# phuang1024/Starst3r

Hardware: AMD Instinct MI355X
Metric: 3DGS train iters/sec @ 1M Gaussians, 8x1080p views (higher is better)
Workload: dtype f32

## Files before the change

### starst3r_amd/csrc/adam.hip

```cpp
#include "per_view.h"

struct AdamK {
    float step_size, bc2_sqrt, w1, w2, b2, eps;
};

#define ADAM_SKIP(count_dev, count_cap, status_dev) \
    (((count_dev) && (uint32_t)(count_dev)[0] > (count_cap)) || ((status_dev) && (status_dev)[0] != 0))

__device__ __forceinline__ float* adam_param(int64_t i, int64_t N, float* means, float* quats, float* scales,
                                             float* opacities, float* sh, int sh_stride) {
    if (i < 3 * N) return means + i;
    if (i < 7 * N) return quats + (i - 3 * N);
    if (i < 10 * N) return scales + (i - 7 * N);
    if (i < 11 * N) return opacities + (i - 10 * N);
    const int64_t j = i - 11 * N;
    const int64_t g = j / 12;
    return sh + g * sh_stride + (j - g * 12);
}

__global__ __launch_bounds__(256) void k_adam(int64_t N, float* __restrict__ means, float* __restrict__ quats,
                                              float* __restrict__ scales, float* __restrict__ opacities,
                                              float* __restrict__ sh, int sh_stride,
                                              const float* __restrict__ grads, float* __restrict__ m,
                                              float* __restrict__ v, AdamK k, const int32_t* __restrict__ count_dev,
                                              uint32_t count_cap, const int32_t* __restrict__ status_dev, int64_t i0,
                                              int64_t i1, int64_t g0, int64_t g1,
                                              float* __restrict__ pstage, const float* __restrict__ gstage,
                                              float* __restrict__ grads_out) {
    if (ADAM_SKIP(count_dev, count_cap, status_dev)) return;
    const bool by_gaussian = g1 - g0 < N || gstage;
    const int64_t n = g1 - g0;
    const int64_t total = by_gaussian ? 23 * n : i1 - i0;
    const int64_t stride = (int64_t)gridDim.x * blockDim.x;
    for (int64_t j = (int64_t)blockIdx.x * blockDim.x + threadIdx.x; j < total; j += stride) {
        int64_t i;
        if (by_gaussian) {
            if (j < 3 * n) i = 3 * g0 + j;
            else if (j < 7 * n) i = 3 * N + 4 * g0 + (j - 3 * n);
            else if (j < 10 * n) i = 7 * N + 3 * g0 + (j - 7 * n);
            else if (j < 11 * n) i = 10 * N + g0 + (j - 10 * n);
            else i = 11 * N + 12 * g0 + (j - 11 * n);
        } else {
            i = i0 + j;
        }
        float* p = adam_param(i, N, means, quats, scales, opacities, sh, sh_stride);
        float gi;
        if (gstage) { gi = gstage[23 * g0 + j]; grads_out[i] = gi; }
        else gi = grads[i];
        const float mi = fmaf(k.w1, gi - m[i], m[i]);
        const float vi = v[i] * k.b2 + (k.w2 * gi) * gi;
        m[i] = mi; v[i] = vi;
        const float denom = sqrtf(vi) / k.bc2_sqrt + k.eps;
        const float pn = *p - k.step_size * (mi / denom);
        *p = pn;
        if (pstage) pstage[i] = pn;
    }
}

__global__ __launch_bounds__(256) void k_adam4(int64_t N, float* __restrict__ means, float* __restrict__ quats,
                                               float* __restrict__ scales, float* __restrict__ opacities,
                                               float* __restrict__ sh, int sh_stride,
                                               const float* __restrict__ grads, float* __restrict__ m,
                                               float* __restrict__ v, AdamK k, const int32_t* __restrict__ count_dev,
                                               uint32_t count_cap, const int32_t* __restrict__ status_dev, int64_t i0,
                                               int64_t i1, float* __restrict__ pstage) {
    if (ADAM_SKIP(count_dev, count_cap, status_dev)) return;
    const int64_t total4 = (i1 - i0) >> 2;
    const int64_t stride = (int64_t)gridDim.x * blockDim.x;
    for (int64_t j = (int64_t)blockIdx.x * blockDim.x + threadIdx.x; j < total4; j += stride) {
        const int64_t i = i0 + 4 * j;
        float4* p = reinterpret_cast<float4*>(adam_param(i, N, means, quats, scales, opacities, sh, sh_stride));
        const float4 g4 = *reinterpret_cast<const float4*>(grads + i);
        float4 m4 = *reinterpret_cast<float4*>(m + i), v4 = *reinterpret_cast<float4*>(v + i), p4 = *p;
        const float gi[4] = {g4.x, g4.y, g4.z, g4.w};
        float mi[4] = {m4.x, m4.y, m4.z, m4.w}, vi[4] = {v4.x, v4.y, v4.z, v4.w}, pi[4] = {p4.x, p4.y, p4.z, p4.w};
#pragma unroll
        for (int q = 0; q < 4; ++q) {
            mi[q] = fmaf(k.w1, gi[q] - mi[q], mi[q]);
            vi[q] = vi[q] * k.b2 + (k.w2 * gi[q]) * gi[q];
            const float denom = sqrtf(vi[q]) / k.bc2_sqrt + k.eps;
            pi[q] = pi[q] - k.step_size * (mi[q] / denom);
        }
        *reinterpret_cast<float4*>(m + i) = make_float4(mi[0], mi[1], mi[2], mi[3]);
        *reinterpret_cast<float4*>(v + i) = make_float4(vi[0], vi[1], vi[2], vi[3]);
        const float4 pn = make_float4(pi[0], pi[1], pi[2], pi[3]);
        *p = pn;
        if (pstage) *reinterpret_cast<float4*>(pstage + i) = pn;
    }
}

__global__ __launch_bounds__(256) void k_params_from_stage(int64_t N, float* __restrict__ means, float* __restrict__ quats,
                                                           float* __restrict__ scales, float* __restrict__ opacities,
                                                           float* __restrict__ sh, int sh_stride,
                                                           const float* __restrict__ pstage, int64_t i0, int64_t i1,
                                                           int64_t lim, const int32_t* __restrict__ count_dev,
                                                           uint32_t count_cap, const int32_t* __restrict__ status_dev) {
    if (ADAM_SKIP(count_dev, count_cap, status_dev)) return;
    const int64_t stride = (int64_t)gridDim.x * blockDim.x;
    for (int64_t i = (int64_t)blockIdx.x * blockDim.x + threadIdx.x; i < lim; i += stride) {
        if (i >= i0 && i < i1) continue;
        *adam_param(i, N, means, quats, scales, opacities, sh, sh_stride) = pstage[i];
    }
}

__global__ __launch_bounds__(256) void k_params_from_peers(int64_t N, float* __restrict__ means, float* __restrict__ quats,
                                                           float* __restrict__ scales, float* __restrict__ opacities,
                                                           float* __restrict__ sh, int sh_stride,
                                                           const float* const* __restrict__ tab, int r, int64_t q,
                                                           int64_t lim, const int32_t* __restrict__ status_dev) {
    if (status_dev && status_dev[0] != 0) return;
    const int64_t stride = (int64_t)gridDim.x * blockDim.x;
    for (int64_t i = (int64_t)blockIdx.x * blockDim.x + threadIdx.x; i < lim; i += stride) {
        const int p = (int)(i / q);
        if (p == r) continue;
        *adam_param(i, N, means, quats, scales, opacities, sh, sh_stride) =
            __uint_as_float(__hip_atomic_load(reinterpret_cast<const unsigned*>(tab[p] + i), __ATOMIC_RELAXED, __HIP_MEMORY_SCOPE_SYSTEM));
    }
}

int st3r_params_from_peers_impl(hipStream_t s, int N, float* means, float* quats, float* scales, float* opacities,
                                float* sh, int sh_stride, const float* const* tab, int r, int64_t q, int64_t lim,
                                const int32_t* status_dev) {
    if (lim <= 0 || q <= 0) return ST3R_OK;
    int blocks = ceil_div(lim, 256);
    if (blocks > 256 * 16) blocks = 256 * 16;
    hipLaunchKernelGGL(k_params_from_peers, dim3(blocks), dim3(256), 0, s, (int64_t)N, means, quats, scales, opacities, sh,
                       sh_stride, tab, r, q, lim, status_dev);
    LAUNCH_CHECK();
    return ST3R_OK;
}

static AdamK adam_constants(double lr, double b1, double b2, double eps, int step) {
    AdamK k;
    const double bc1 = 1.0 - pow(b1, (double)step), bc2 = 1.0 - pow(b2, (double)step);
    k.step_size = (float)(lr / bc1);
    k.bc2_sqrt = (float)sqrt(bc2);
    k.w1 = (float)(1.0 - b1); k.w2 = (float)(1.0 - b2); k.b2 = (float)b2; k.eps = (float)eps;
    return k;
}

int st3r_adam_impl(hipStream_t s, int N, float* means, float* quats, float* scales, float* opacities, float* sh,
                   int sh_stride, const float* grads, float* m, float* v, double lr, double b1, double b2,
                   double eps, int step, const int32_t* count_dev, uint32_t count_cap, const int32_t* status_dev, int64_t i0,
                   int64_t i1, int64_t g0, int64_t g1, float* pstage, const float* gstage, float* grads_out) {
    if (N == 0) return ST3R_OK;
    if (i0 < 0) { i0 = 0; i1 = 23 * (int64_t)N; }
    if (g1 < 0) { g0 = 0; g1 = N; }
    const AdamK k = adam_constants(lr, b1, b2, eps, step);
    const int64_t total = (g1 - g0 < N) ? 23 * (g1 - g0) : i1 - i0;
    if (total <= 0) return ST3R_OK;
    const bool contiguous = !(g1 - g0 < N) && !gstage;
#ifndef ADAM_NO_VEC
    if (contiguous && N % 4 == 0 && i0 % 4 == 0 && (i1 - i0) % 4 == 0 && sh_stride % 4 == 0 &&
        aligned16(means, quats, scales, opacities, sh, grads, m, v, pstage)) {
        int blocks4 = ceil_div(total / 4, 256);
        if (blocks4 > 256 * 16) blocks4 = 256 * 16;
        hipLaunchKernelGGL(k_adam4, dim3(blocks4), dim3(256), 0, s, (int64_t)N, means, quats, scales, opacities, sh,
                           sh_stride, grads, m, v, k, count_dev, count_cap, status_dev, i0, i1, pstage);
        LAUNCH_CHECK();
        return ST3R_OK;
    }
#endif
    int blocks = ceil_div(total, 256);
    if (blocks > 256 * 16) blocks = 256 * 16;
    hipLaunchKernelGGL(k_adam, dim3(blocks), dim3(256), 0, s, (int64_t)N, means, quats, scales, opacities, sh,
                       sh_stride, grads, m, v, k, count_dev, count_cap, status_dev, i0, i1, g0, g1, pstage, gstage, grads_out);
    LAUNCH_CHECK();
    return ST3R_OK;
}

int st3r_params_from_stage_impl(hipStream_t s, int N, float* means, float* quats, float* scales, float* opacities,
// ... 54 lines not shown
```

### starst3r_amd/csrc/comm.hip

```cpp
#include <dlfcn.h>

#include <vector>

#include <rccl/rccl.h>

#include <chrono>
#include <thread>

#include "stages.h"

namespace {
struct RcclApi {
    void* handle;
    ncclResult_t (*get_unique_id)(ncclUniqueId*);
    ncclResult_t (*comm_init_rank)(ncclComm_t*, int, ncclUniqueId, int);
    ncclResult_t (*comm_destroy)(ncclComm_t);
    ncclResult_t (*all_reduce)(const void*, void*, size_t, ncclDataType_t, ncclRedOp_t, ncclComm_t, hipStream_t);
    ncclResult_t (*reduce_scatter)(const void*, void*, size_t, ncclDataType_t, ncclRedOp_t, ncclComm_t, hipStream_t);
    ncclResult_t (*all_gather)(const void*, void*, size_t, ncclDataType_t, ncclComm_t, hipStream_t);
    ncclResult_t (*group_start)();
    ncclResult_t (*group_end)();
    const char* (*get_error_string)(ncclResult_t);
};

// ... 319 lines not shown
    }
    __syncthreads();
    if (p == 0 && status_out) *status_out = accumulate ? (*status_out | s_any) : s_any;
    __threadfence_system();
}

__device__ __forceinline__ float peer_load(const float* p) {
    return __uint_as_float(__hip_atomic_load(reinterpret_cast<const unsigned*>(p), __ATOMIC_RELAXED, __HIP_MEMORY_SCOPE_SYSTEM));
}
__global__ __launch_bounds__(256) void k_xreduce(const float* const* __restrict__ grad_tab, int w, int r, int64_t i0,
                                                 int64_t i1, int64_t t0, int64_t t1, float* __restrict__ out) {
    const int64_t n = (i1 - i0) + (t1 - t0);
    const int64_t stride = (int64_t)gridDim.x * blockDim.x;
    for (int64_t j = (int64_t)blockIdx.x * blockDim.x + threadIdx.x; j < n; j += stride) {
        const int64_t i = j < i1 - i0 ? i0 + j : t0 + (j - (i1 - i0));
        float acc = 0.f;
        for (int p = 0; p < w; ++p) {
            const float v = p == r ? grad_tab[p][i] : peer_load(grad_tab[p] + i);
            acc = p == 0 ? v : acc + v;
        }
        out[i] = acc;
    }
}

ST3R_EXPORT int st3r_gs_train_step(st3r_ctx* ctx, void* stream, int N, int C, float* means, float* quats, float* scales,
                                   float* opacities, float* sh, int sh_stride, const float* viewmats, const float* Ks,
                                   const float* campos, const float* gt_images, int width, int height, float ssim_fac,
                                   float opac_fac, float scale_fac, float* grads, float* m, float* v, double lr,
                                   double beta1, double beta2, double eps, int step, float* loss_out,
                                   int64_t* stats_host) {
    ARG_CHECK(ctx && grads && m && v && step >= 1 && N > 0);
    hipStream_t s = (hipStream_t)stream;
    if (!ctx->comm) {
        int rc = st3r_gs_train_fwd_bwd(ctx, stream, N, C, means, quats, scales, opacities, sh, sh_stride, viewmats, Ks,
                                       campos, gt_images, width, height, ssim_fac, opac_fac, scale_fac, grads, loss_out,
                                       stats_host);
        if (rc) return rc;
        return st3r_adam_step(ctx, stream, N, means, quats, scales, opacities, sh, sh_stride, grads, m, v, lr, beta1, beta2,
                              eps, step);
    }
    RcclApi* api = rccl_api();
    if (!api) return ST3R_ERR_HIP;
    ncclComm_t comm = (ncclComm_t)ctx->comm;
    int rc = st3r_peer_status_settle(ctx);
    if (rc) return rc;
    if (ctx->comm_broken) {
        st3r_set_error("this communicator lost lockstep in an earlier step (a device-side barrier timed out): no further "
                       "step is exchanged over it");
        return ST3R_ERR_PEER;
    }
    const int mode = ctx->exchange;
    int32_t* counts = nullptr;
    rc = st3r_counts_buffer(ctx, s, &counts);
    if (rc) return rc;
    if (!ctx->peer_event) HIP_TRY(hipEventCreateWithFlags(&ctx->peer_event, hipEventDisableTiming));
    const int K = (mode == ST3R_EXCHANGE_RANGES && N >= 4096) ? EXCH_RANGES_K : 1;
    if (mode == ST3R_EXCHANGE_RANGES) {
        rc = ensure_comm_stream(ctx);
        if (rc) return rc;
        ctx->n_ranges = K;
    }
    XWindow* xw = nullptr;
    if (mode == ST3R_EXCHANGE_DIRECT) {
        rc = xwin_ensure(ctx, api, s, (int64_t)23 * N);
        if (rc) return rc;
        xw = (XWindow*)ctx->xwin;
    }
    float* const grads_local = xw ? xw->grad : grads;
    int rc_local = (ctx->debug_flags & 2048)
                       ? (st3r_set_error("debug flag 2048: simulated failure of this rank's step"), ST3R_ERR_NOMEM)
// ... 129 lines not shown
```

### starst3r_amd/csrc/fused_step.hip

```cpp
#include "radix_sort.h"
#include "stages.h"

int st3r_count_settle(st3r_ctx* ctx) {
    if (!ctx->count_pending) return ST3R_OK;
    HIP_TRY(hipEventSynchronize(ctx->count_event));
    ctx->count_pending = 0;
    const int64_t n = (int64_t)((int32_t*)(ctx->pinned + 8))[0];
    if (n < 0) {
        ctx->isect_hint = 0;
        ctx->view_chunks = (ctx->view_chunks > 0 ? ctx->view_chunks : 1) * 2;
        st3r_set_error("the previous step produced more than 2^31 tile intersections: its gradients were incomplete -- "
                       "repeat it (st3r_gs_train_fwd_bwd / st3r_gs_train_step now walk the views in %d chunks)",
                       ctx->view_chunks);
        return ST3R_ERR_CAPACITY;
    }
    if (n > ctx->count_cap) {
        ctx->isect_hint = 0;
        st3r_set_error("the previous step produced %lld tile intersections, more than the %lld its buffers were sized "
                       "for from the step before (+25 %%): its gradients were incomplete and st3r_adam_step / "
                       "st3r_gs_train_step did NOT apply them (the update is guarded on the device) -- repeat that step",
                       (long long)n, (long long)ctx->count_cap);
        return ST3R_ERR_CAPACITY;
    }
    ctx->isect_hint = n;
// ... 228 lines not shown
        rc = st3r_loss_impl(ctx, s, ro.C, ro.H, ro.W, ex.exposure ? im.exposed : im.rgb, b.gt, 1.0f - ssim_fac, ssim_fac,
                            b.sums, im.v_rgb, sums_cleared, lw);
    if (!rc && ex.exposure)
        rc = st3r_exposure_bwd_impl(ctx, s, ro.C, ro.H, ro.W, im.rgb, ex.exposure, im.v_rgb, im.v_rgb, ex.v_exposure);
    if (!rc && dp.prior)
        rc = st3r_depth_prior_loss_impl(ctx, s, ro.C, ro.H, ro.W, im.depth, im.alpha, dp.prior, dp.weight, dp.norm, 1, dp.fac,
                                        b.dp_sums, 1, im.v_depth, im.v_alpha);
    st3r_prof_end(ctx, s, STG_LOSS);
    return rc;
}

static int blend_backward(st3r_ctx* ctx, hipStream_t s, const RasterOut& ro, const StepImages& im, bool need_pairs,
                          st3r_vtile_ref* slots, float* v_pairs) {
    RasterOut rb = ro;
    if (ctx->debug_flags & 2) { rb.rects = nullptr; rb.rectbase = nullptr; }
    const bool eio = true;
    st3r_prof_begin(ctx, s, STG_BLEND_BWD);
    int rc = st3r_blend_bwd_impl(ctx, s, rb, im.alpha, im.last, im.v_rgb, im.v_alpha, nullptr, eio, slots);
    if (!rc && need_pairs) {
        ARENA_GET(SLOT_VSPLATS_D, float, ro.n_pairs * ST3R_SPLAT_STRIDE, v_pairs_d);
        rc = st3r_blend_depth_bwd_impl(ctx, s, rb, im.alpha, im.last, im.v_depth, v_pairs_d, eio);
        if (!rc) {
            if (slots->vtile) rc = st3r_gather_vtile_impl(s, ro.n_pairs, slots, v_pairs);
            else HIP_TRY(hipMemsetAsync(v_pairs, 0, sizeof(float) * ST3R_SPLAT_STRIDE * (size_t)ro.n_pairs, s));
        }
        if (!rc) rc = st3r_add_pairs_impl(s, ro.n_pairs, v_pairs, v_pairs_d);
    }
    st3r_prof_end(ctx, s, STG_BLEND_BWD);
    return rc;
}

static int project_backward(st3r_ctx* ctx, hipStream_t s, const GsParams& g, const GsViews& v, const RasterOut& ro,
                            const LossFacs& f, const float* v_pairs, const st3r_vtile_ref* slots, bool accumulate,
                            float* grads) {
    ctx->ranges_recorded = 0;
    if (!(ctx->n_ranges > 1 && ctx->comm_stream))
        return st3r_project_sh_bwd_impl(s, g, v, 0.3f, ro.splats, v_pairs, (float)v.C, f.opac, f.scale, grads, accumulate, 0,
                                        -1, false, slots);
    ARENA_GET(SLOT_GSTAGE, float, (int64_t)23 * g.N, gstage);
    const int K = ctx->n_ranges;
    for (int j = 0; j < K; ++j) {
        const int g0 = (int)((int64_t)g.N * j / K), g1 = (int)((int64_t)g.N * (j + 1) / K);
        int rc = st3r_project_sh_bwd_impl(s, g, v, 0.3f, ro.splats, v_pairs, (float)v.C, f.opac, f.scale, gstage, accumulate,
                                          g0, g1, true, slots);
        if (rc) return rc;
        HIP_TRY(hipEventRecord(ctx->ev_range_bwd[j], s));
    }
    ctx->ranges_recorded = K;
    return ST3R_OK;
}

static int pose_backward(st3r_ctx* ctx, hipStream_t s, const GsParams& g, const GsViews& v, const RasterOut& ro,
                         const float* v_pairs, float* v_viewmats) {
    return st3r_gs_viewmat_bwd(ctx, s, g.N, v.C, g.means, g.quats, g.scales, g.sh, g.sh_stride, v.viewmats, v.Ks, v.campos,
                               v.W, v.H, 0.3f, ro.splats, v_pairs, v_viewmats);
}

static int train_views(st3r_ctx* ctx, hipStream_t s, const GsParams& g, const ViewBatch& b, const LossFacs& f,
                       double* reg_sums, bool allow_async, bool accumulate, float* grads, RasterOut* ro_out) {
    const GsViews& v = b.v;
    DepthPrior dp{};
    int rc = b.dp_sums ? st3r_depth_prior_for(ctx, s, b.gt, v.C, v.H, v.W, &dp) : ST3R_OK;
    if (rc) return rc;
    ExposureReg ex{};
    if (b.exposure) st3r_exposure_for(ctx, b.gt, v.C, v.H, v.W, &ex);
    LossWeight lw{};
    if (b.weighted) rc = st3r_loss_weight_for(ctx, s, b.gt, v.C, v.H, v.W, &lw);
    if (rc) return rc;
    const bool need_pairs = dp.prior != nullptr;
    RasterOut& ro = *ro_out;
    rc = rasterize_front(ctx, s, g, v, reg_sums, 1, nullptr, allow_async, &ro, b.sums);
    if (rc) return rc;
    StepImages im;
    rc = step_images(ctx, ro, need_pairs, ex.exposure != nullptr, &im);
    if (rc) return rc;
    float* const v_Ks = st3r_intrinsics_grad_for(ctx, b.gt, v.C, v.H, v.W);
    float* v_pairs = nullptr;
    if (need_pairs || b.v_viewmats || v_Ks) {
        ARENA_GET(SLOT_VSPLATS, float, ro.n_pairs * ST3R_SPLAT_STRIDE, vp);
        v_pairs = vp;
    }
    rc = forward_and_losses(ctx, s, ro, b, f.ssim, true, dp, ex, lw, im);
    if (rc) return rc;
    st3r_vtile_ref slots{};
    rc = blend_backward(ctx, s, ro, im, need_pairs, &slots, v_pairs);
    if (rc) return rc;
    st3r_prof_begin(ctx, s, STG_PROJECT_BWD);
    rc = project_backward(ctx, s, g, v, ro, f, need_pairs ? v_pairs : nullptr, need_pairs ? nullptr : &slots, accumulate,
                          grads);
    if (!rc && need_pairs && b.v_viewmats) rc = pose_backward(ctx, s, g, v, ro, v_pairs, b.v_viewmats);
    if (!rc && need_pairs) rc = st3r_gs_depth_bwd(ctx, s, g.N, v.C, g.means, v.viewmats, ro.splats, v_pairs, grads, b.v_viewmats);
    st3r_prof_end(ctx, s, STG_PROJECT_BWD);
    if (!rc && !need_pairs && (b.v_viewmats || v_Ks)) {
        rc = st3r_gather_vtile_impl(s, ro.n_pairs, &slots, v_pairs);
        if (!rc && b.v_viewmats) rc = pose_backward(ctx, s, g, v, ro, v_pairs, b.v_viewmats);
    }
    if (!rc && v_Ks)
        rc = st3r_gs_intrinsics_bwd(ctx, s, g.N, v.C, g.means, g.quats, g.scales, v.viewmats, v.Ks, v.W, v.H, 0.3f,
                                    ro.splats, v_pairs, v_Ks);
    return rc;
}

static int train_chunks(st3r_ctx* ctx, hipStream_t s, const GsParams& g, const ViewBatch& all, const LossFacs& f,
                        double* reg_sums, double* reg_scratch, bool want_stats, float* grads, int* chunks, int64_t stats[3]) {
    const int C = all.v.C;
    for (;;) {
        int rc = ST3R_OK;
        stats[0] = stats[1] = stats[2] = 0;
        bool first = true;
        for (int k = 0; k < *chunks && !rc; ++k) {
            const int c0 = (int)((int64_t)k * C / *chunks), c1 = (int)((int64_t)(k + 1) * C / *chunks);
            if (c1 == c0) continue;
            RasterOut ro;
            rc = train_views(ctx, s, g, all.slice(c0, c1), f, first ? reg_sums : reg_scratch,
                             !want_stats && *chunks == 1 && !ctx->comm, !first, grads, &ro);
            if (!rc) { stats[0] += ro.n_visible; stats[1] += ro.n_records; stats[2] += ro.n_isects_ref; }
            first = false;
        }
        if (rc == ST3R_SPLIT_VIEWS && *chunks < C) {
            *chunks = *chunks * 2 < C ? *chunks * 2 : C;
            continue;
        }
        return rc == ST3R_SPLIT_VIEWS ? ST3R_ERR_INVALID : rc;
    }
}

int st3r_train_fwd_bwd_impl(st3r_ctx* ctx, hipStream_t s, const GsParams& g, const GsViews& v, const float* gt_images,
                            float ssim_fac, float opac_fac, float scale_fac, float* grads, float* loss_out,
                            int64_t* stats_host, float* v_viewmats) {
    const int N = g.N, C = v.C;
    ARG_CHECK(ctx && N > 0 && C > 0 && C <= ST3R_MAX_VIEWS && v.W > 0 && v.H > 0 && g.sh_stride >= 12);
    ARG_CHECK((int64_t)N * C < 2147483647LL);
    ARG_CHECK(g.means && g.quats && g.scales && g.opacities && g.sh && v.viewmats && v.Ks && v.campos && gt_images && grads &&
              loss_out);
    ARENA_GET(SLOT_SMALL, double, 2 * (size_t)C + 12, small);
    double* sums = small;
    double* reg_sums = small + 2 * C;
    double* dp_sums = nullptr;
    DepthPrior dp;
    int rc = st3r_depth_prior_for(ctx, s, gt_images, C, v.H, v.W, &dp);
    if (rc) return rc;
    if (dp.prior) {
        if (ctx->comm) {
            st3r_set_error("a depth prior is registered and a communicator is attached -- the depth term is not "
                           "supported in view-sharded training (clear it with st3r_ctx_set_depth_prior(ctx, NULL, ...))");
            return ST3R_ERR_INVALID;
        }
        ARENA_GET(SLOT_DPRIOR_SUMS, double, (size_t)C, ds);
        dp_sums = ds;
    }
    ExposureReg ex;
    st3r_exposure_for(ctx, gt_images, C, v.H, v.W, &ex);
    if (ex.exposure && ctx->comm) {
        st3r_set_error("exposures are registered and a communicator is attached -- per-view exposures are not supported "
                       "in view-sharded training (clear them with st3r_ctx_set_exposure(ctx, NULL, ...))");
        return ST3R_ERR_INVALID;
    }
    if (ctx->comm && st3r_intrinsics_grad_for(ctx, gt_images, C, v.H, v.W)) {
        st3r_set_error("an intrinsics gradient is registered and a communicator is attached -- intrinsics refinement is "
                       "not supported in view-sharded training (clear it with st3r_ctx_set_intrinsics_grad(ctx, NULL, ...))");
        return ST3R_ERR_INVALID;
    }
    LossWeight lw;
    rc = st3r_loss_weight_for(ctx, s, gt_images, C, v.H, v.W, &lw);
    if (rc) return rc;
    if (lw.weight && ctx->comm) {
        st3r_set_error("loss weights are registered and a communicator is attached -- per-pixel loss weights are not "
                       "supported in view-sharded training (clear them with st3r_ctx_set_loss_weight(ctx, NULL, ...))");
        return ST3R_ERR_INVALID;
    }
    st3r_prof_next_step(ctx);
    rc = st3r_count_settle(ctx);
    if (rc) return rc;
    int chunks = ctx->view_chunks > 0 ? ctx->view_chunks : 1;
    if ((ctx->debug_flags & 32) && chunks < 2) chunks = 2;
    if (chunks > C) chunks = C;
    int64_t stats[3];
    rc = train_chunks(ctx, s, g, ViewBatch{v, gt_images, sums, dp_sums, v_viewmats, ex.exposure != nullptr, lw.weight != nullptr},
                      LossFacs{ssim_fac, opac_fac, scale_fac},
                      reg_sums, reg_sums + 4, stats_host != nullptr, grads, &chunks, stats);
    if (rc) return rc;
    if (chunks > 1) ctx->view_chunks = chunks;
    rc = finalize_loss(s, C, v.H, v.W, sums, reg_sums, ssim_fac, (double)C, (double)opac_fac / N,
                       (double)scale_fac / (3.0 * N), loss_out, dp_sums, dp, lw);
    if (rc) return rc;
    if (stats_host) {
        stats_host[0] = stats[0]; stats_host[1] = stats[1]; stats_host[2] = st3r_ctx_arena_bytes(ctx);
        stats_host[3] = stats[2];
    }
    return ST3R_OK;
}

ST3R_EXPORT int st3r_gs_train_fwd_bwd(st3r_ctx* ctx, void* stream, int N, int C, const float* means,
                                      const float* quats, const float* scales, const float* opacities,
                                      const float* sh, int sh_stride, const float* viewmats, const float* Ks,
                                      const float* campos, const float* gt_images, int width, int height,
                                      float ssim_fac, float opac_fac, float scale_fac, float* grads,
                                      float* loss_out, int64_t* stats_host) {
    return st3r_train_fwd_bwd_impl(ctx, (hipStream_t)stream, GsParams{N, means, quats, scales, opacities, sh, sh_stride},
                                   GsViews{C, width, height, viewmats, Ks, campos}, gt_images, ssim_fac, opac_fac,
                                   scale_fac, grads, loss_out, stats_host, nullptr);
}

ST3R_EXPORT int st3r_gs_raster_train(st3r_ctx* ctx, void* stream, int N, int C, const float* records,
                                     const float* gt_images, int width, int height, float ssim_fac,
                                     float* v_records, float* loss_out, int64_t* stats_host) {
    ARG_CHECK(ctx && N > 0 && C > 0 && width > 0 && height > 0 && records && gt_images && v_records && loss_out);
    ARG_CHECK(C <= ST3R_MAX_VIEWS && (int64_t)N * C < 2147483647LL);
    hipStream_t s = (hipStream_t)stream;
    ARENA_GET(SLOT_SMALL, double, 2 * (size_t)C + 8, sums);
    double* reg_sums = sums + 2 * C;
    const ViewBatch b{GsViews{C, width, height}, gt_images, sums, nullptr, nullptr, false, false};
    HIP_TRY(hipMemsetAsync(reg_sums, 0, sizeof(double) * 4, s));
// ... 85 lines not shown
```

### starst3r_amd/csrc/gs_project_bwd.hip

```cpp
#include "stages.h"
#include "blend_common.h"
#include "project_common.h"

#ifndef GATHER_WIDE_ABOVE
#define GATHER_WIDE_ABOVE 6
#endif

template <bool GATHER>
__global__ __launch_bounds__(256) __attribute__((amdgpu_waves_per_eu(4))) void k_project_sh_bwd(
    int N, int C, const float* __restrict__ means, const float* __restrict__ quats,
    const float* __restrict__ scales, const float* __restrict__ opacities, const float* __restrict__ sh,
    int sh_stride, const float* __restrict__ viewmats, const float* __restrict__ Ks,
    const float* __restrict__ campos, int W, int H, float eps2d, const float4* __restrict__ splats,
    const float4* __restrict__ v_splats, float reg_o_k, float reg_s_k, float* __restrict__ grads, int accumulate,
    int g_begin, int g_end, int range_major, const int32_t* __restrict__ cum, const float* __restrict__ vtile, int stamp,
    unsigned vt_cap, const uint32_t* __restrict__ touch) {
    extern __shared__ float cam[];
    constexpr int ROW = ACC_VALS;
    __shared__ float sVal[GATHER ? 256 * ROW : 1];
    __shared__ float sAcc[GATHER ? 256 * ROW : 1];
    __shared__ int sStart[GATHER ? 4 * 65 : 1];
    for (int c = threadIdx.x; c < C; c += blockDim.x) {
        float* o = cam + c * CAM_STRIDE;
        const float* V = viewmats + 16 * c;
        for (int k = 0; k < 12; ++k) o[k] = V[k];
        const float* K = Ks + 9 * c;
        float fx = K[0], fy = K[4], cx = K[2], cy = K[5];
        o[12] = fx; o[13] = fy; o[14] = cx; o[15] = cy;
        float tan_fovx = 0.5f * (float)W / fx;
        float tan_fovy = 0.5f * (float)H / fy;
        o[16] = ((float)W - cx) / fx + 0.3f * tan_fovx;
        o[17] = cx / fx + 0.3f * tan_fovx;
        o[18] = ((float)H - cy) / fy + 0.3f * tan_fovy;
        o[19] = cy / fy + 0.3f * tan_fovy;
        o[20] = campos[3 * c]; o[21] = campos[3 * c + 1]; o[22] = campos[3 * c + 2];
    }
    __syncthreads();
    const int gbase = g_begin + blockIdx.x * blockDim.x;
    const bool valid = gbase + (int)threadIdx.x < g_end;
    if (!GATHER && !valid) return;
    const int g = valid ? gbase + (int)threadIdx.x : g_end - 1;

    const float mx = means[3 * g], my = means[3 * g + 1], mz = means[3 * g + 2];
    const float opac = opacities[g];
    float qw = quats[4 * g], qx = quats[4 * g + 1], qy = quats[4 * g + 2], qz = quats[4 * g + 3];
    const float s0 = scales[3 * g], s1 = scales[3 * g + 1], s2 = scales[3 * g + 2];
    float k[12];
    const float* kp = sh + (int64_t)g * sh_stride;
#pragma unroll
// ... 220 lines not shown
    }

    if (GATHER && !valid) return;
    float Rq[9], M[9];
    asm volatile("" : "+v"(qw), "+v"(qx), "+v"(qy), "+v"(qz));
    rot_and_m(Rq, M);
    const float W9[9] = {vSw[0], vSw[1], vSw[2], vSw[1], vSw[3], vSw[4], vSw[2], vSw[4], vSw[5]};
    float vM[9];
#pragma unroll
    for (int r = 0; r < 3; ++r)
#pragma unroll
        for (int s = 0; s < 3; ++s)
            vM[r * 3 + s] = 2.0f * (W9[r * 3] * M[s] + W9[r * 3 + 1] * M[3 + s] + W9[r * 3 + 2] * M[6 + s]);
    float v_scale[3], vR[9];
#pragma unroll
    for (int s = 0; s < 3; ++s) {
        v_scale[s] = Rq[s] * vM[s] + Rq[3 + s] * vM[3 + s] + Rq[6 + s] * vM[6 + s];
        vR[s] = vM[s] * sc[s]; vR[3 + s] = vM[3 + s] * sc[s]; vR[6 + s] = vM[6 + s] * sc[s];
    }
    float vq0 = 2.0f * (qx * (vR[7] - vR[5]) + qy * (vR[2] - vR[6]) + qz * (vR[3] - vR[1]));
    float vq1 = 2.0f * (-2.0f * qx * (vR[4] + vR[8]) + qy * (vR[3] + vR[1]) + qz * (vR[6] + vR[2]) + qw * (vR[7] - vR[5]));
    float vq2 = 2.0f * (qx * (vR[3] + vR[1]) - 2.0f * qy * (vR[0] + vR[8]) + qz * (vR[7] + vR[5]) + qw * (vR[2] - vR[6]));
    float vq3 = 2.0f * (qx * (vR[6] + vR[2]) + qy * (vR[7] + vR[5]) - 2.0f * qz * (vR[0] + vR[4]) + qw * (vR[3] - vR[1]));
    const float dq = vq0 * qw + vq1 * qx + vq2 * qy + vq3 * qz;
    vq0 = (vq0 - dq * qw) * inv_norm; vq1 = (vq1 - dq * qx) * inv_norm;
    vq2 = (vq2 - dq * qy) * inv_norm; vq3 = (vq3 - dq * qz) * inv_norm;

    const float sg = 1.0f / (1.0f + __expf(-opac));
    v_opac += reg_o_k * sg * (1.0f - sg);
    v_scale[0] += reg_s_k * __expf(s0);
    v_scale[1] += reg_s_k * __expf(s1);
    v_scale[2] += reg_s_k * __expf(s2);

    const int64_t Nl = range_major ? g_end - g_begin : N;
    float* gb = range_major ? grads + (int64_t)23 * g_begin : grads;
    const int gw = range_major ? g - g_begin : g;
    float* gm = gb; float* gq = gb + 3 * Nl; float* gs = gb + 7 * Nl;
    float* go = gb + 10 * Nl; float* gsh = gb + 11 * Nl;
    if (accumulate) {
        v_mean[0] += gm[3 * gw]; v_mean[1] += gm[3 * gw + 1]; v_mean[2] += gm[3 * gw + 2];
        vq0 += gq[4 * gw]; vq1 += gq[4 * gw + 1]; vq2 += gq[4 * gw + 2]; vq3 += gq[4 * gw + 3];
        v_scale[0] += gs[3 * gw]; v_scale[1] += gs[3 * gw + 1]; v_scale[2] += gs[3 * gw + 2];
        v_opac += go[gw];
#pragma unroll
        for (int i = 0; i < 12; ++i) v_k[i] += gsh[(int64_t)gw * 12 + i];
    }
    gm[3 * gw] = v_mean[0]; gm[3 * gw + 1] = v_mean[1]; gm[3 * gw + 2] = v_mean[2];
    gq[4 * gw] = vq0; gq[4 * gw + 1] = vq1; gq[4 * gw + 2] = vq2; gq[4 * gw + 3] = vq3;
    gs[3 * gw] = v_scale[0]; gs[3 * gw + 1] = v_scale[1]; gs[3 * gw + 2] = v_scale[2];
    go[gw] = v_opac;
#pragma unroll
    for (int i = 0; i < 12; ++i) gsh[(int64_t)gw * 12 + i] = v_k[i];
}

int st3r_project_sh_bwd_impl(hipStream_t s, const GsParams& g, const GsViews& v, float eps2d, const float* splats,
                             const float* v_splats, float reg_views, float opac_fac, float scale_fac, float* grads,
                             bool accumulate, int g_begin, int g_end, bool range_major, const st3r_vtile_ref* slots) {
    const int N = g.N, C = v.C;
    if (g_end < 0) g_end = N;
    if (N == 0 || g_end <= g_begin) return ST3R_OK;
    float reg_o_k = reg_views * opac_fac / (float)N;
    float reg_s_k = reg_views * scale_fac / (3.0f * (float)N);
    size_t shmem = (size_t)C * CAM_STRIDE * sizeof(float);
    if (slots)
        hipLaunchKernelGGL(k_project_sh_bwd<true>, dim3(ceil_div(g_end - g_begin, 256)), dim3(256), shmem, s, N, C, g.means,
                           g.quats, g.scales, g.opacities, g.sh, g.sh_stride, v.viewmats, v.Ks, v.campos, v.W, v.H, eps2d,
                           (const float4*)splats, (const float4*)nullptr, reg_o_k, reg_s_k, grads, accumulate ? 1 : 0, g_begin,
                           g_end, range_major ? 1 : 0, slots->cum, slots->vtile, slots->stamp, slots->vt_cap, slots->touch);
    else
        hipLaunchKernelGGL(k_project_sh_bwd<false>, dim3(ceil_div(g_end - g_begin, 256)), dim3(256), shmem, s, N, C, g.means,
                           g.quats, g.scales, g.opacities, g.sh, g.sh_stride, v.viewmats, v.Ks, v.campos, v.W, v.H, eps2d,
                           (const float4*)splats, (const float4*)v_splats, reg_o_k, reg_s_k, grads, accumulate ? 1 : 0, g_begin,
                           g_end, range_major ? 1 : 0, (const int32_t*)nullptr, (const float*)nullptr, 0, 0u, (const uint32_t*)nullptr);
    LAUNCH_CHECK();
    return ST3R_OK;
}

ST3R_EXPORT int st3r_gs_project_sh_bwd(st3r_ctx* ctx, void* stream, int N, int C, const float* means,
                                       const float* quats, const float* scales, const float* opacities,
                                       const float* sh, int sh_stride, const float* viewmats, const float* Ks,
                                       const float* campos, int width, int height, float eps2d,
                                       const float* splats, const float* v_splats, float reg_views,
                                       float opac_fac, float scale_fac, float* grads) {
    ARG_CHECK(ctx && N >= 0 && C > 0 && C <= ST3R_MAX_VIEWS && sh_stride >= 12);
    ARG_CHECK(means && quats && scales && opacities && sh && viewmats && Ks && campos && splats && v_splats && grads);
    return st3r_project_sh_bwd_impl((hipStream_t)stream, GsParams{N, means, quats, scales, opacities, sh, sh_stride},
                                    GsViews{C, width, height, viewmats, Ks, campos}, eps2d, splats, v_splats, reg_views, opac_fac, scale_fac,
                                    grads, false, 0, -1, false, nullptr);
}
```

### starst3r_amd/csrc/stages.h

```cpp
#pragma once
#include "common.h"

struct GsParams {
    int N;
    const float *means, *quats, *scales, *opacities, *sh;
    int sh_stride;
};

struct GsViews {
    int C, W, H;
    const float *viewmats, *Ks, *campos;
    GsViews slice(int c0, int c1) const { return {c1 - c0, W, H, viewmats + 16 * c0, Ks + 9 * c0, campos + 3 * c0}; }
};

struct RasterOut {
    int C, W, H, tile_w, tile_h;
    const float* splats; const int32_t *offsets, *flat, *cum; const uint64_t *rects, *rectbase;
    int tight;
    int64_t n_pairs;
    int64_t n_isects, n_records, n_isects_ref, n_visible;
};

static inline RasterOut stage_lists(int C, int W, int H, int tile_w, int tile_h, const float* splats, const int32_t* offsets,
                                    const int32_t* flat, int64_t n_isects, const int32_t* cum = nullptr,
                                    int64_t n_pairs = 0) {
    return RasterOut{C, W, H, tile_w, tile_h, splats, offsets, flat, cum, nullptr, nullptr, 0, n_pairs, n_isects, n_isects,
                     n_isects, -1};
}

struct DepthPrior { const float* prior; const float* weight; const double* norm; float fac; };

struct ExposureReg { const float* exposure; float* v_exposure; };

struct LossWeight { const float* weight = nullptr; const double* norm = nullptr; int norm_stride = 0; int sums_stride = 2; };

int st3r_counts_buffer(st3r_ctx* ctx, hipStream_t s, int32_t** out);
int st3r_count_settle(st3r_ctx* ctx);
int st3r_train_fwd_bwd_impl(st3r_ctx* ctx, hipStream_t s, const GsParams& g, const GsViews& v, const float* gt_images,
                            float ssim_fac, float opac_fac, float scale_fac, float* grads, float* loss_out,
                            int64_t* stats_host, float* v_viewmats);
int st3r_peer_status_settle(st3r_ctx* ctx);

int st3r_project_impl(st3r_ctx* ctx, hipStream_t s, const GsParams& g, const GsViews& v, int tile_size, float eps2d,
                      float near_plane, float far_plane, float radius_clip, float* splats, int32_t* tiles_per_gauss,
                      double* reg_sums, uint64_t* depth_keys, int32_t* depth_vals, int tight, uint32_t key_base, void* rects,
                      int rect32, int reg_overwrite, double* zero_ptr, int zero_n, uint32_t* krange);
int st3r_project_sh_bwd_impl(hipStream_t s, const GsParams& g, const GsViews& v, float eps2d, const float* splats,
                             const float* v_splats, float reg_views, float opac_fac, float scale_fac, float* grads,
                             bool accumulate, int g_begin, int g_end, bool range_major, const st3r_vtile_ref* slots);

int st3r_isect_scan_impl(st3r_ctx* ctx, hipStream_t s, int64_t n_pairs, const int32_t* tiles, int32_t* cum,
                         int64_t* n_isects_host, const void* pack_rects, int rect32, uint64_t* pack_out,
                         int32_t** total_dev_out, int32_t* total_copy, int32_t* total_host);
int st3r_scan_tiles(int64_t n);
void st3r_emit_grid(int N, int C, int* bpc, int* grid, int* self_base);
void st3r_isect_constants(int64_t out[5]);
int st3r_isect_emit_chain_impl(st3r_ctx* ctx, hipStream_t s, int N, int C, const int32_t* perm, const void* rects,
                               int rect32, int tile_w, int tile_h, uint32_t* tile_keys, int32_t* vals, int64_t cap,
                               int band_tile, const int32_t* n_dev, const uint32_t** band_table);
int st3r_records_prepare_impl(hipStream_t s, int N, int C, const float* splats, int tile_size, int tile_w, int tile_h,
                              int tight, int32_t* tiles, uint64_t* depth_keys, int32_t* depth_vals, uint32_t key_base,
                              void* rects, int rect32);
int st3r_isect_offsets32_impl(hipStream_t s, int64_t n_isects, const uint32_t* keys, int C, int tile_w, int tile_h,
                              int32_t* offsets, const int32_t* n_dev);
int st3r_sort_tile_end_bit(int end_bit);
int st3r_sort_tile_impl(st3r_ctx* ctx, hipStream_t s, int64_t n, int end_bit, uint32_t* keys_in, int32_t* vals_in,
                        uint32_t* keys_out, int32_t* vals_out, const int32_t* n_dev);
int st3r_sort_tile_banded(int end_bit, int debug_flags);

int st3r_blend_fwd_impl(st3r_ctx* ctx, hipStream_t s, const RasterOut& ro, float* rgb, float* alpha, int32_t* last_ids,
                        bool for_backward, bool end_in_offsets);
int st3r_blend_fwd_cells_impl(st3r_ctx* ctx, hipStream_t s, const RasterOut& ro, float* rgb, float* alpha,
                              int32_t* last_ids, uint64_t* cmask, int64_t cmask_words, int32_t* tile_nb);
int st3r_blend_bwd_impl(st3r_ctx* ctx, hipStream_t s, const RasterOut& ro, const float* alpha, const int32_t* last_ids,
                        const float* v_rgb, const float* v_alpha, float* v_splats, bool end_in_offsets,
                        st3r_vtile_ref* defer);
int st3r_gather_vtile_impl(hipStream_t s, int64_t n_pairs, const st3r_vtile_ref* slots, float* v_splats);
int st3r_blend_depth_fwd_impl(st3r_ctx* ctx, hipStream_t s, const RasterOut& ro, const int32_t* last_ids, float* depth,
                              bool end_in_offsets);
int st3r_blend_depth_bwd_impl(st3r_ctx* ctx, hipStream_t s, const RasterOut& ro, const float* alpha,
                              const int32_t* last_ids, const float* v_depth, float* v_splats, bool end_in_offsets);
int st3r_add_pairs_impl(hipStream_t s, int64_t n_pairs, float* a, const float* b);
// ... 32 lines not shown
```

Before: 195.8.

## Fuse Adam optimizer update into project/SH backward kernel tail

On the single-device, single-chunk path without pose or intrinsics gradients, the per-Gaussian backward kernel now applies the Adam update directly to its 23 gradient values. It loads m and v, updates them along with the parameters in registers, and writes everything back, so the separate Adam kernel launch is skipped. This removes a full re-read of the gradients and parameters from memory. In exchange the fused kernel holds more live values, which can raise register pressure or lower occupancy, and it adds a guard check inside the kernel. The Adam math was moved into a shared header and explicit FMAs were pinned so both paths compute the update the same way.

```diff
diff --git a/starst3r_amd/csrc/adam.hip b/starst3r_amd/csrc/adam.hip
--- a/starst3r_amd/csrc/adam.hip
+++ b/starst3r_amd/csrc/adam.hip
@@ -1,11 +1,5 @@
 #include "per_view.h"
-
-struct AdamK {
-    float step_size, bc2_sqrt, w1, w2, b2, eps;
-};
-
-#define ADAM_SKIP(count_dev, count_cap, status_dev) \
-    (((count_dev) && (uint32_t)(count_dev)[0] > (count_cap)) || ((status_dev) && (status_dev)[0] != 0))
+#include "adam_update.h"
 
 __device__ __forceinline__ float* adam_param(int64_t i, int64_t N, float* means, float* quats, float* scales,
                                              float* opacities, float* sh, int sh_stride) {
@@ -47,11 +41,9 @@
         float gi;
         if (gstage) { gi = gstage[23 * g0 + j]; grads_out[i] = gi; }
         else gi = grads[i];
-        const float mi = fmaf(k.w1, gi - m[i], m[i]);
-        const float vi = v[i] * k.b2 + (k.w2 * gi) * gi;
+        float mi = m[i], vi = v[i], pn = *p;
+        adam_scalar(k, gi, mi, vi, pn);
         m[i] = mi; v[i] = vi;
-        const float denom = sqrtf(vi) / k.bc2_sqrt + k.eps;
-        const float pn = *p - k.step_size * (mi / denom);
         *p = pn;
         if (pstage) pstage[i] = pn;
     }
@@ -75,12 +67,7 @@
         const float gi[4] = {g4.x, g4.y, g4.z, g4.w};
         float mi[4] = {m4.x, m4.y, m4.z, m4.w}, vi[4] = {v4.x, v4.y, v4.z, v4.w}, pi[4] = {p4.x, p4.y, p4.z, p4.w};
 #pragma unroll
-        for (int q = 0; q < 4; ++q) {
-            mi[q] = fmaf(k.w1, gi[q] - mi[q], mi[q]);
-            vi[q] = vi[q] * k.b2 + (k.w2 * gi[q]) * gi[q];
-            const float denom = sqrtf(vi[q]) / k.bc2_sqrt + k.eps;
-            pi[q] = pi[q] - k.step_size * (mi[q] / denom);
-        }
+        for (int q = 0; q < 4; ++q) adam_scalar(k, gi[q], mi[q], vi[q], pi[q]);
         *reinterpret_cast<float4*>(m + i) = make_float4(mi[0], mi[1], mi[2], mi[3]);
         *reinterpret_cast<float4*>(v + i) = make_float4(vi[0], vi[1], vi[2], vi[3]);
         const float4 pn = make_float4(pi[0], pi[1], pi[2], pi[3]);
@@ -128,15 +115,6 @@
                        sh_stride, tab, r, q, lim, status_dev);
     LAUNCH_CHECK();
     return ST3R_OK;
-}
-
-static AdamK adam_constants(double lr, double b1, double b2, double eps, int step) {
-    AdamK k;
-    const double bc1 = 1.0 - pow(b1, (double)step), bc2 = 1.0 - pow(b2, (double)step);
-    k.step_size = (float)(lr / bc1);
-    k.bc2_sqrt = (float)sqrt(bc2);
-    k.w1 = (float)(1.0 - b1); k.w2 = (float)(1.0 - b2); k.b2 = (float)b2; k.eps = (float)eps;
-    return k;
 }
 
 int st3r_adam_impl(hipStream_t s, int N, float* means, float* quats, float* scales, float* opacities, float* sh,
diff --git a/starst3r_amd/csrc/adam_update.h b/starst3r_amd/csrc/adam_update.h
--- /dev/null
+++ b/starst3r_amd/csrc/adam_update.h
@@ -0,0 +1,28 @@
+#pragma once
+#include <hip/hip_runtime.h>
+#include <math.h>
+#include <stdint.h>
+
+struct AdamK {
+    float step_size, bc2_sqrt, w1, w2, b2, eps;
+};
+
+#define ADAM_SKIP(count_dev, count_cap, status_dev) \
+    (((count_dev) && (uint32_t)(count_dev)[0] > (count_cap)) || ((status_dev) && (status_dev)[0] != 0))
+
+static inline AdamK adam_constants(double lr, double b1, double b2, double eps, int step) {
+    AdamK k;
+    const double bc1 = 1.0 - pow(b1, (double)step), bc2 = 1.0 - pow(b2, (double)step);
+    k.step_size = (float)(lr / bc1);
+    k.bc2_sqrt = (float)sqrt(bc2);
+    k.w1 = (float)(1.0 - b1); k.w2 = (float)(1.0 - b2); k.b2 = (float)b2; k.eps = (float)eps;
+    return k;
+}
+
+__device__ __forceinline__ void adam_scalar(const AdamK& k, float g, float& m, float& v, float& p) {
+#pragma clang fp contract(off)
+    m = fmaf(k.w1, g - m, m);
+    v = fmaf(k.b2, v, (k.w2 * g) * g);
+    const float denom = sqrtf(v) / k.bc2_sqrt + k.eps;
+    p = fmaf(-k.step_size, m / denom, p);
+}
diff --git a/starst3r_amd/csrc/comm.hip b/starst3r_amd/csrc/comm.hip
--- a/starst3r_amd/csrc/comm.hip
+++ b/starst3r_amd/csrc/comm.hip
@@ -375,10 +375,13 @@
     ARG_CHECK(ctx && grads && m && v && step >= 1 && N > 0);
     hipStream_t s = (hipStream_t)stream;
     if (!ctx->comm) {
-        int rc = st3r_gs_train_fwd_bwd(ctx, stream, N, C, means, quats, scales, opacities, sh, sh_stride, viewmats, Ks,
-                                       campos, gt_images, width, height, ssim_fac, opac_fac, scale_fac, grads, loss_out,
-                                       stats_host);
+        AdamTail tail{m, v, lr, beta1, beta2, eps, step, nullptr, 0xFFFFFFFFu, false};
+        int rc = st3r_train_fwd_bwd_impl(ctx, s, GsParams{N, means, quats, scales, opacities, sh, sh_stride},
+                                         GsViews{C, width, height, viewmats, Ks, campos}, gt_images, ssim_fac, opac_fac,
+                                         scale_fac, grads, loss_out, stats_host, nullptr,
+                                         (ctx->debug_flags & 4096) ? nullptr : &tail);
         if (rc) return rc;
+        if (tail.applied) return ST3R_OK;
         return st3r_adam_step(ctx, stream, N, means, quats, scales, opacities, sh, sh_stride, grads, m, v, lr, beta1, beta2,
                               eps, step);
     }
diff --git a/starst3r_amd/csrc/fused_step.hip b/starst3r_amd/csrc/fused_step.hip
--- a/starst3r_amd/csrc/fused_step.hip
+++ b/starst3r_amd/csrc/fused_step.hip
@@ -284,11 +284,13 @@
 
 static int project_backward(st3r_ctx* ctx, hipStream_t s, const GsParams& g, const GsViews& v, const RasterOut& ro,
                             const LossFacs& f, const float* v_pairs, const st3r_vtile_ref* slots, bool accumulate,
-                            float* grads) {
+                            float* grads, AdamTail* adam) {
     ctx->ranges_recorded = 0;
-    if (!(ctx->n_ranges > 1 && ctx->comm_stream))
+    if (!(ctx->n_ranges > 1 && ctx->comm_stream)) {
+        if (adam) st3r_adam_guard(ctx, &adam->count_dev, &adam->count_cap);
         return st3r_project_sh_bwd_impl(s, g, v, 0.3f, ro.splats, v_pairs, (float)v.C, f.opac, f.scale, grads, accumulate, 0,
-                                        -1, false, slots);
+                                        -1, false, slots, adam);
+    }
     ARENA_GET(SLOT_GSTAGE, float, (int64_t)23 * g.N, gstage);
     const int K = ctx->n_ranges;
     for (int j = 0; j < K; ++j) {
@@ -309,7 +311,8 @@
 }
 
 static int train_views(st3r_ctx* ctx, hipStream_t s, const GsParams& g, const ViewBatch& b, const LossFacs& f,
-                       double* reg_sums, bool allow_async, bool accumulate, float* grads, RasterOut* ro_out) {
+                       double* reg_sums, bool allow_async, bool accumulate, float* grads, RasterOut* ro_out,
+                       AdamTail* adam) {
     const GsViews& v = b.v;
     DepthPrior dp{};
     int rc = b.dp_sums ? st3r_depth_prior_for(ctx, s, b.gt, v.C, v.H, v.W, &dp) : ST3R_OK;
@@ -337,9 +340,10 @@
     st3r_vtile_ref slots{};
     rc = blend_backward(ctx, s, ro, im, need_pairs, &slots, v_pairs);
     if (rc) return rc;
+    if (need_pairs || b.v_viewmats || v_Ks) adam = nullptr;
     st3r_prof_begin(ctx, s, STG_PROJECT_BWD);
     rc = project_backward(ctx, s, g, v, ro, f, need_pairs ? v_pairs : nullptr, need_pairs ? nullptr : &slots, accumulate,
-                          grads);
+                          grads, adam);
     if (!rc && need_pairs && b.v_viewmats) rc = pose_backward(ctx, s, g, v, ro, v_pairs, b.v_viewmats);
     if (!rc && need_pairs) rc = st3r_gs_depth_bwd(ctx, s, g.N, v.C, g.means, v.viewmats, ro.splats, v_pairs, grads, b.v_viewmats);
     st3r_prof_end(ctx, s, STG_PROJECT_BWD);
@@ -354,7 +358,8 @@
 }
 
 static int train_chunks(st3r_ctx* ctx, hipStream_t s, const GsParams& g, const ViewBatch& all, const LossFacs& f,
-                        double* reg_sums, double* reg_scratch, bool want_stats, float* grads, int* chunks, int64_t stats[3]) {
+                        double* reg_sums, double* reg_scratch, bool want_stats, float* grads, int* chunks, int64_t stats[3],
+                        AdamTail* adam) {
     const int C = all.v.C;
     for (;;) {
         int rc = ST3R_OK;
@@ -365,7 +370,8 @@
             if (c1 == c0) continue;
             RasterOut ro;
             rc = train_views(ctx, s, g, all.slice(c0, c1), f, first ? reg_sums : reg_scratch,
-                             !want_stats && *chunks == 1 && !ctx->comm, !first, grads, &ro);
+                             !want_stats && *chunks == 1 && !ctx->comm, !first, grads, &ro,
+                             *chunks == 1 && !ctx->comm ? adam : nullptr);
             if (!rc) { stats[0] += ro.n_visible; stats[1] += ro.n_records; stats[2] += ro.n_isects_ref; }
             first = false;
         }
@@ -379,7 +385,7 @@
 
 int st3r_train_fwd_bwd_impl(st3r_ctx* ctx, hipStream_t s, const GsParams& g, const GsViews& v, const float* gt_images,
                             float ssim_fac, float opac_fac, float scale_fac, float* grads, float* loss_out,
-                            int64_t* stats_host, float* v_viewmats) {
+                            int64_t* stats_host, float* v_viewmats, AdamTail* adam) {
     const int N = g.N, C = v.C;
     ARG_CHECK(ctx && N > 0 && C > 0 && C <= ST3R_MAX_VIEWS && v.W > 0 && v.H > 0 && g.sh_stride >= 12);
     ARG_CHECK((int64_t)N * C < 2147483647LL);
@@ -430,7 +436,7 @@
     int64_t stats[3];
     rc = train_chunks(ctx, s, g, ViewBatch{v, gt_images, sums, dp_sums, v_viewmats, ex.exposure != nullptr, lw.weight != nullptr},
                       LossFacs{ssim_fac, opac_fac, scale_fac},
-                      reg_sums, reg_sums + 4, stats_host != nullptr, grads, &chunks, stats);
+                      reg_sums, reg_sums + 4, stats_host != nullptr, grads, &chunks, stats, adam);
     if (rc) return rc;
     if (chunks > 1) ctx->view_chunks = chunks;
     rc = finalize_loss(s, C, v.H, v.W, sums, reg_sums, ssim_fac, (double)C, (double)opac_fac / N,
diff --git a/starst3r_amd/csrc/gs_project_bwd.hip b/starst3r_amd/csrc/gs_project_bwd.hip
--- a/starst3r_amd/csrc/gs_project_bwd.hip
+++ b/starst3r_amd/csrc/gs_project_bwd.hip
@@ -1,20 +1,30 @@
 #include "stages.h"
 #include "blend_common.h"
 #include "project_common.h"
+#include "adam_update.h"
 
 #ifndef GATHER_WIDE_ABOVE
 #define GATHER_WIDE_ABOVE 6
 #endif
 
-template <bool GATHER>
+struct AdamTailK {
+    AdamK k;
+    const int32_t* count_dev; uint32_t count_cap;
+};
+template <bool WRITTEN> struct ParamPtr { using type = const float* __restrict__; };
+template <> struct ParamPtr<true> { using type = float* __restrict__; };
+
+template <bool GATHER, bool ADAM = false>
 __global__ __launch_bounds__(256) __attribute__((amdgpu_waves_per_eu(4))) void k_project_sh_bwd(
-    int N, int C, const float* __restrict__ means, const float* __restrict__ quats,
-    const float* __restrict__ scales, const float* __restrict__ opacities, const float* __restrict__ sh,
+    int N, int C, typename ParamPtr<ADAM>::type means, typename ParamPtr<ADAM>::type quats,
+    typename ParamPtr<ADAM>::type scales, typename ParamPtr<ADAM>::type opacities, typename ParamPtr<ADAM>::type sh,
     int sh_stride, const float* __restrict__ viewmats, const float* __restrict__ Ks,
     const float* __restrict__ campos, int W, int H, float eps2d, const float4* __restrict__ splats,
     const float4* __restrict__ v_splats, float reg_o_k, float reg_s_k, float* __restrict__ grads, int accumulate,
     int g_begin, int g_end, int range_major, const int32_t* __restrict__ cum, const float* __restrict__ vtile, int stamp,
-    unsigned vt_cap, const uint32_t* __restrict__ touch) {
+    unsigned vt_cap, const uint32_t* __restrict__ touch, float* __restrict__ adam_m, float* __restrict__ adam_v,
+    AdamTailK ad) {
+    static_assert(GATHER || !ADAM, "the Adam tail belongs to the fused training calls");
     extern __shared__ float cam[];
     constexpr int ROW = ACC_VALS;
     __shared__ float sVal[GATHER ? 256 * ROW : 1];
@@ -301,12 +311,27 @@
     v_scale[1] += reg_s_k * __expf(s1);
     v_scale[2] += reg_s_k * __expf(s2);
 
+    float am[ADAM ? 23 : 1], av[ADAM ? 23 : 1], qraw[4] = {0.f, 0.f, 0.f, 0.f};
+    int64_t ga = g;
+    if constexpr (ADAM) {
+        asm volatile("" ::: "memory");
+        asm volatile("" : "+v"(ga));
+        const int64_t at[5] = {3 * ga, 3 * (int64_t)N + 4 * ga, 7 * (int64_t)N + 3 * ga, 10 * (int64_t)N + ga, 11 * (int64_t)N + 12 * ga};
+        constexpr int first[6] = {0, 3, 7, 10, 11, 23};
+#pragma unroll
+        for (int b = 0; b < 5; ++b)
+#pragma unroll
+            for (int j = first[b]; j < first[b + 1]; ++j) { am[j] = adam_m[at[b] + (j - first[b])]; av[j] = adam_v[at[b] + (j - first[b])]; }
+#pragma unroll
+        for (int j = 0; j < 4; ++j) qraw[j] = quats[4 * ga + j];
+        __builtin_amdgcn_sched_barrier(0);
+    }
     const int64_t Nl = range_major ? g_end - g_begin : N;
     float* gb = range_major ? grads + (int64_t)23 * g_begin : grads;
     const int gw = range_major ? g - g_begin : g;
     float* gm = gb; float* gq = gb + 3 * Nl; float* gs = gb + 7 * Nl;
     float* go = gb + 10 * Nl; float* gsh = gb + 11 * Nl;
-    if (accumulate) {
+    if (!ADAM && accumulate) {
         v_mean[0] += gm[3 * gw]; v_mean[1] += gm[3 * gw + 1]; v_mean[2] += gm[3 * gw + 2];
         vq0 += gq[4 * gw]; vq1 += gq[4 * gw + 1]; vq2 += gq[4 * gw + 2]; vq3 += gq[4 * gw + 3];
         v_scale[0] += gs[3 * gw]; v_scale[1] += gs[3 * gw + 1]; v_scale[2] += gs[3 * gw + 2];
@@ -320,27 +345,63 @@
     go[gw] = v_opac;
 #pragma unroll
     for (int i = 0; i < 12; ++i) gsh[(int64_t)gw * 12 + i] = v_k[i];
+
+    if constexpr (ADAM) {
+        if (ADAM_SKIP(ad.count_dev, ad.count_cap, (const int32_t*)nullptr)) return;
+        const float gr[23] = {v_mean[0], v_mean[1], v_mean[2], vq0, vq1, vq2, vq3, v_scale[0], v_scale[1], v_scale[2], v_opac,
+                              v_k[0], v_k[1], v_k[2], v_k[3], v_k[4], v_k[5], v_k[6], v_k[7], v_k[8], v_k[9], v_k[10], v_k[11]};
+        float pr[23] = {mx, my, mz, qraw[0], qraw[1], qraw[2], qraw[3], s0, s1, s2, opac,
+                        k[0], k[1], k[2], k[3], k[4], k[5], k[6], k[7], k[8], k[9], k[10], k[11]};
+#pragma unroll
+        for (int j = 0; j < 23; ++j) adam_scalar(ad.k, gr[j], am[j], av[j], pr[j]);
+        const int64_t at[5] = {3 * ga, 3 * Nl + 4 * ga, 7 * Nl + 3 * ga, 10 * Nl + ga, 11 * Nl + 12 * ga};
+        float* const pt[5] = {means + 3 * ga, quats + 4 * ga, scales + 3 * ga, opacities + ga, sh + ga * sh_stride};
+        constexpr int first[6] = {0, 3, 7, 10, 11, 23};
+#pragma unroll
+        for (int b = 0; b < 5; ++b)
+#pragma unroll
+            for (int j = first[b]; j < first[b + 1]; ++j) {
+                adam_m[at[b] + (j - first[b])] = am[j]; adam_v[at[b] + (j - first[b])] = av[j];
+                pt[b][j - first[b]] = pr[j];
+            }
+    }
 }
 
 int st3r_project_sh_bwd_impl(hipStream_t s, const GsParams& g, const GsViews& v, float eps2d, const float* splats,
                              const float* v_splats, float reg_views, float opac_fac, float scale_fac, float* grads,
-                             bool accumulate, int g_begin, int g_end, bool range_major, const st3r_vtile_ref* slots) {
+                             bool accumulate, int g_begin, int g_end, bool range_major, const st3r_vtile_ref* slots,
+                             AdamTail* adam) {
     const int N = g.N, C = v.C;
     if (g_end < 0) g_end = N;
     if (N == 0 || g_end <= g_begin) return ST3R_OK;
     float reg_o_k = reg_views * opac_fac / (float)N;
     float reg_s_k = reg_views * scale_fac / (3.0f * (float)N);
     size_t shmem = (size_t)C * CAM_STRIDE * sizeof(float);
+    const dim3 grid(ceil_div(g_end - g_begin, 256)), block(256);
+    const AdamTailK no_tail{};
+    if (adam && slots && !accumulate && !range_major && g_begin == 0 && g_end == N) {
+        const AdamTailK ad{adam_constants(adam->lr, adam->b1, adam->b2, adam->eps, adam->step), adam->count_dev, adam->count_cap};
+        hipLaunchKernelGGL((k_project_sh_bwd<true, true>), grid, block, shmem, s, N, C, const_cast<float*>(g.means),
+                           const_cast<float*>(g.quats), const_cast<float*>(g.scales), const_cast<float*>(g.opacities),
+                           const_cast<float*>(g.sh), g.sh_stride, v.viewmats, v.Ks, v.campos, v.W, v.H, eps2d,
+                           (const float4*)splats, (const float4*)nullptr, reg_o_k, reg_s_k, grads, 0, g_begin, g_end, 0,
+                           slots->cum, slots->vtile, slots->stamp, slots->vt_cap, slots->touch, adam->m, adam->v, ad);
+        LAUNCH_CHECK();
+        adam->applied = true;
+        return ST3R_OK;
+    }
     if (slots)
-        hipLaunchKernelGGL(k_project_sh_bwd<true>, dim3(ceil_div(g_end - g_begin, 256)), dim3(256), shmem, s, N, C, g.means,
+        hipLaunchKernelGGL(k_project_sh_bwd<true>, grid, block, shmem, s, N, C, g.means,
                            g.quats, g.scales, g.opacities, g.sh, g.sh_stride, v.viewmats, v.Ks, v.campos, v.W, v.H, eps2d,
                            (const float4*)splats, (const float4*)nullptr, reg_o_k, reg_s_k, grads, accumulate ? 1 : 0, g_begin,
-                           g_end, range_major ? 1 : 0, slots->cum, slots->vtile, slots->stamp, slots->vt_cap, slots->touch);
+                           g_end, range_major ? 1 : 0, slots->cum, slots->vtile, slots->stamp, slots->vt_cap, slots->touch,
+                           (float*)nullptr, (float*)nullptr, no_tail);
     else
-        hipLaunchKernelGGL(k_project_sh_bwd<false>, dim3(ceil_div(g_end - g_begin, 256)), dim3(256), shmem, s, N, C, g.means,
+        hipLaunchKernelGGL(k_project_sh_bwd<false>, grid, block, shmem, s, N, C, g.means,
                            g.quats, g.scales, g.opacities, g.sh, g.sh_stride, v.viewmats, v.Ks, v.campos, v.W, v.H, eps2d,
                            (const float4*)splats, (const float4*)v_splats, reg_o_k, reg_s_k, grads, accumulate ? 1 : 0, g_begin,
-                           g_end, range_major ? 1 : 0, (const int32_t*)nullptr, (const float*)nullptr, 0, 0u, (const uint32_t*)nullptr);
+                           g_end, range_major ? 1 : 0, (const int32_t*)nullptr, (const float*)nullptr, 0, 0u, (const uint32_t*)nullptr,
+                           (float*)nullptr, (float*)nullptr, no_tail);
     LAUNCH_CHECK();
     return ST3R_OK;
 }
diff --git a/starst3r_amd/csrc/stages.h b/starst3r_amd/csrc/stages.h
--- a/starst3r_amd/csrc/stages.h
+++ b/starst3r_amd/csrc/stages.h
@@ -34,11 +34,19 @@
 
 struct LossWeight { const float* weight = nullptr; const double* norm = nullptr; int norm_stride = 0; int sums_stride = 2; };
 
+struct AdamTail {
+    float *m, *v;
+    double lr, b1, b2, eps;
+    int step;
+    const int32_t* count_dev; uint32_t count_cap;
+    bool applied;
+};
+
 int st3r_counts_buffer(st3r_ctx* ctx, hipStream_t s, int32_t** out);
 int st3r_count_settle(st3r_ctx* ctx);
 int st3r_train_fwd_bwd_impl(st3r_ctx* ctx, hipStream_t s, const GsParams& g, const GsViews& v, const float* gt_images,
                             float ssim_fac, float opac_fac, float scale_fac, float* grads, float* loss_out,
-                            int64_t* stats_host, float* v_viewmats);
+                            int64_t* stats_host, float* v_viewmats, AdamTail* adam = nullptr);
 int st3r_peer_status_settle(st3r_ctx* ctx);
 
 int st3r_project_impl(st3r_ctx* ctx, hipStream_t s, const GsParams& g, const GsViews& v, int tile_size, float eps2d,
@@ -47,7 +55,8 @@
                       int rect32, int reg_overwrite, double* zero_ptr, int zero_n, uint32_t* krange);
 int st3r_project_sh_bwd_impl(hipStream_t s, const GsParams& g, const GsViews& v, float eps2d, const float* splats,
                              const float* v_splats, float reg_views, float opac_fac, float scale_fac, float* grads,
-                             bool accumulate, int g_begin, int g_end, bool range_major, const st3r_vtile_ref* slots);
+                             bool accumulate, int g_begin, int g_end, bool range_major, const st3r_vtile_ref* slots,
+                             AdamTail* adam = nullptr);
 
 int st3r_isect_scan_impl(st3r_ctx* ctx, hipStream_t s, int64_t n_pairs, const int32_t* tiles, int32_t* cum,
                          int64_t* n_isects_host, const void* pack_rects, int rect32, uint64_t* pack_out,
```

New measurement: 199.3, median of 4. About the same (+1.8%).
